# darchr/DLRM.jl

Measured on NVIDIA B200. Metric: dlrm_train_samples_per_sec, higher is better.
Workload: dtype f32 (3xTF32 interaction forward)

## Files before the change

### dlrm_jl_b200/_lib.py

```python
from __future__ import annotations

import ctypes as C
import os
from typing import Optional

HERE = os.path.dirname(os.path.abspath(__file__))
LIB_PATH = os.path.join(HERE, "lib", "libdlrm_b200.so")

OK, EINVAL, ECUDA, ENOMEM, EOOB, ESTATE, ENCCL = 0, 1, 2, 3, 4, 5, 6
_STATUS_NAMES = {EINVAL: "DLRMB_EINVAL", ECUDA: "DLRMB_ECUDA", ENOMEM: "DLRMB_ENOMEM",
                 EOOB: "DLRMB_EOOB", ESTATE: "DLRMB_ESTATE", ENCCL: "DLRMB_ENCCL"}


class DLRMB200Error(RuntimeError):
    def __init__(self, status: int, message: str):
        super().__init__(f"{_STATUS_NAMES.get(status, status)}: {message}")
        self.status = status


_i32, _i64, _f32, _vp = C.c_int32, C.c_int64, C.c_float, C.c_void_p
_idx_args = [_vp, _i32, _i32, _i32, _i32]
_idx_mp_args = [_vp, _i32, _i32, _i32, C.POINTER(_i32)]

SIGNATURES = {
    "dlrmb_abi_version": (_i32, []),
    "dlrmb_last_error": (C.c_char_p, []),
    "dlrmb_launch_count": (_i64, []),
    "dlrmb_set_option": (_i32, [C.c_char_p, _i64]),
    "dlrmb_get_option": (_i32, [C.c_char_p, C.POINTER(_i64)]),
    "dlrmb_clock_buffer_bytes": (_i64, []),
    "dlrmb_clock_kernels": (_i32, []),
    "dlrmb_clock_enable": (_i32, [_vp]),
    "dlrmb_tables_create": (_i32, [_i32, _i32, C.POINTER(_i64), _i32, _i64, C.POINTER(_vp)]),
    "dlrmb_tables_create_ex": (_i32, [_i32, _i32, C.POINTER(_i64), _i32, _i64, _i32, C.POINTER(_vp)]),
    "dlrmb_tables_elem_bytes": (_i32, [_vp]),
    "dlrmb_tables_reserve": (_i32, [_vp, _i64]),
    "dlrmb_tables_destroy": (_i32, [_vp]),
    "dlrmb_tables_info": (_i32, [_vp, C.POINTER(_i32), C.POINTER(_i32), C.POINTER(_i64), C.POINTER(_i64)]),
    "dlrmb_tables_upload": (_i32, [_vp, _i32, _vp]),
    "dlrmb_tables_download": (_i32, [_vp, _i32, _vp]),
    "dlrmb_tables_device_ptr": (_i32, [_vp, _i32, C.POINTER(_vp)]),
    "dlrmb_tables_init_uniform": (_i32, [_vp, C.c_uint64, _vp]),
    "dlrmb_tables_sync": (_i32, [_vp]),
    "dlrmb_embedding_fwd": (_i32, [_vp, *_idx_args, _vp, _i32, _i32, _vp]),
    "dlrmb_embedding_fwd_sort": (_i32, [_vp, *_idx_args, _vp, _i32, _i32, _vp]),
    "dlrmb_interaction_fwd": (_i32, [_i32, _vp, _vp, _i32, _i32, _i32, _i32, _vp, _vp]),
    "dlrmb_interaction_bwd": (_i32, [_i32, _vp, _vp, _i32, _i32, _i32, _i32, _vp, _vp, _vp]),
    "dlrmb_embedding_sort": (_i32, [_vp, *_idx_args, _vp]),
    "dlrmb_embedding_update_sorted": (_i32, [_vp, _vp, _i32, _i32, _f32, _vp]),
    "dlrmb_embedding_bwd_sgd": (_i32, [_vp, *_idx_args, _vp, _i32, _i32, _f32, _vp]),
    "dlrmb_sort_dedup_export": (_i32, [_vp, _i32, _vp, _vp, _vp, C.POINTER(_i32)]),
    "dlrmb_check_indices": (_i32, [_vp, *_idx_args, _i32]),
    "dlrmb_bce_sigmoid_fwd_bwd": (_i32, [_i32, _vp, _vp, _i32, _vp, _vp, _vp, _vp, _vp]),
    "dlrmb_xbuf_create": (_i32, [_i32, _i64, C.POINTER(_vp)]),
    "dlrmb_xbuf_destroy": (_i32, [_vp]),
    "dlrmb_xbuf_ptr": (_i32, [_vp, C.POINTER(_vp)]),
    "dlrmb_xbuf_ipc_handle": (_i32, [_vp, _vp]),
    "dlrmb_xbuf_open": (_i32, [_i32, _vp, C.POINTER(_vp)]),
    "dlrmb_xbuf_close": (_i32, [_i32, _vp]),
    "dlrmb_tables_set_slot_map": (_i32, [_vp, C.POINTER(_i32)]),
    "dlrmb_tables_set_dest_map": (_i32, [_vp, C.POINTER(_i32), C.POINTER(_i32), _i32]),
    "dlrmb_embedding_fwd_p2p": (_i32, [_vp, *_idx_args, C.POINTER(_vp), _i32, _i32, _i32, _vp]),
    "dlrmb_embedding_fwd_p2p_sort": (_i32, [_vp, *_idx_args, C.POINTER(_vp), _i32, _i32, _i32, _vp]),
    "dlrmb_embedding_fwd_p2p_mp": (_i32, [_vp, *_idx_mp_args, C.POINTER(_vp), _i32, _i32, _i32, _vp]),
    "dlrmb_embedding_fwd_p2p_sort_mp": (_i32, [_vp, *_idx_mp_args, C.POINTER(_vp), _i32, _i32, _i32, _vp]),
    "dlrmb_peer_barrier": (_i32, [_i32, C.POINTER(_vp), _i32, _i32, _i32, _vp, _vp]),
    "dlrmb_peer_barrier_flag_bytes": (_i64, []),
    "dlrmb_peer_barrier_state_bytes": (_i64, []),
    "dlrmb_peer_allreduce_f32": (_i32, [_i32, C.POINTER(_vp), C.POINTER(_vp), _i32, _i32, _i32, _vp, _vp, _i64, _vp]),
    "dlrmb_indices_scatter_p2p": (_i32, [_i32, _vp, _i32, _i32, _i32, _i32, _vp, _i32, _vp]),
    "dlrmb_indices_scatter_p2p_mp": (_i32, [_i32, _vp, _i32, _i32, _i32, C.POINTER(_i32), _vp, _i32, _vp]),
    "dlrmb_indices_scatter_p2p_mp_list": (_i32, [_i32, _vp, _i32, _i32, _i32, C.POINTER(_i32), _i32, C.POINTER(_i32),
                                                 _vp, _i32, _vp]),
    "dlrmb_interaction_has_warp_path": (_i32, [_i32, _i32]),
    "dlrmb_dense_fwd_bias_act": (_i32, [_i32, _vp, _vp, _i32, _i32, _i32, _vp]),
    "dlrmb_dense_bwd_scratch_floats": (_i64, [_i32]),
    "dlrmb_dense_bwd_act_bias": (_i32, [_i32, _vp, _vp, _i32, _i32, _vp, _vp, _vp, _vp]),
    "dlrmb_interaction_bwd_scatter": (_i32, [_i32, _vp, _vp, _i32, _i32, _i32, _i32, _vp, _i64, _vp, _vp]),
    "dlrmb_interaction_bwd_scatter_cols": (_i32, [_i32, _vp, _vp, _i32, _i32, _i32, _i32, _vp, _i32, _i64, _vp, _vp]),
    "dlrmb_interaction_bwd_dx": (_i32, [_i32, _vp, _vp, _i32, _i32, _i32, _i32, _vp, _vp]),
    "dlrmb_dac_unpack": (_i32, [_i32, _vp, _i32, _vp, _vp, _vp, _vp]),
    "dlrmb_shard_plan": (_i32, [_i32, C.POINTER(_i64), _i32, C.POINTER(_i32)]),
    "dlrmb_shard_plan_mp": (_i32, [_i32, C.POINTER(_i64), C.POINTER(_i32), _i32, C.POINTER(_i32)]),
    "dlrmb_shard_plan_cw": (_i32, [_i32, C.POINTER(_i64), C.POINTER(_i32), _i32, _i32, _i32, C.POINTER(_i32),
                                   C.POINTER(_i32)]),
    "dlrmb_comm_unique_id": (_i32, [_vp]),
    "dlrmb_comm_create": (_i32, [_i32, _vp, _i32, _i32, C.POINTER(_vp)]),
    "dlrmb_comm_destroy": (_i32, [_vp]),
    "dlrmb_comm_info": (_i32, [_vp, C.POINTER(_i32), C.POINTER(_i32)]),
    "dlrmb_comm_a2a_indices": (_i32, [_vp, C.POINTER(_i32), _i32, _vp, _i32, _i32, _i32, _vp, _vp]),
    "dlrmb_comm_a2a_indices_mp": (_i32, [_vp, C.POINTER(_i32), _i32, _vp, _i32, _i32, C.POINTER(_i32), _vp, _vp]),
    "dlrmb_comm_a2a_fwd": (_i32, [_vp, C.POINTER(_i32), _i32, _vp, _i32, _i32, _vp, _vp]),
    "dlrmb_comm_a2a_bwd": (_i32, [_vp, C.POINTER(_i32), _i32, _vp, _i32, _i32, _vp, _vp]),
    "dlrmb_comm_allreduce_f32": (_i32, [_vp, _vp, _i64, _vp]),
    "dlrmb_comm_allgather": (_i32, [_vp, _vp, _vp, _i64, _vp]),
    "dlrmb_embedding_fwd_host": (_i32, [_vp, *_idx_args, _vp, _i32, _i32]),
    "dlrmb_interaction_fwd_host": (_i32, [_vp, _vp, _vp, _i32, _i32, _i32, _i32, _vp]),
    "dlrmb_interaction_bwd_host": (_i32, [_vp, _vp, _vp, _i32, _i32, _i32, _i32, _vp, _vp]),
    "dlrmb_embedding_bwd_sgd_host": (_i32, [_vp, *_idx_args, _vp, _i32, _i32, _f32]),
    "dlrmb_mp_max_tables": (_i32, []),
    "dlrmb_embedding_fwd_mp": (_i32, [_vp, *_idx_mp_args, _vp, _i32, _i32, _vp]),
    "dlrmb_embedding_fwd_sort_mp": (_i32, [_vp, *_idx_mp_args, _vp, _i32, _i32, _vp]),
    "dlrmb_embedding_sort_mp": (_i32, [_vp, *_idx_mp_args, _vp]),
    "dlrmb_embedding_bwd_sgd_mp": (_i32, [_vp, *_idx_mp_args, _vp, _i32, _i32, _f32, _vp]),
    "dlrmb_check_indices_mp": (_i32, [_vp, *_idx_mp_args, _i32]),
    "dlrmb_embedding_fwd_mp_host": (_i32, [_vp, *_idx_mp_args, _vp, _i32, _i32]),
    "dlrmb_embedding_bwd_sgd_mp_host": (_i32, [_vp, *_idx_mp_args, _vp, _i32, _i32, _f32]),
}

_lib: Optional[C.CDLL] = None


def load() -> C.CDLL:
    global _lib
    if _lib is not None:
        return _lib
    if not os.path.exists(LIB_PATH):
        raise DLRMB200Error(
            ESTATE,
            f"{LIB_PATH} not found: build it with `python -m dlrm_jl_b200.csrc.build` "
            "(there is no CPU or PyTorch fallback for this path)")
    lib = C.CDLL(LIB_PATH)
    for name, (res, args) in SIGNATURES.items():
        fn = getattr(lib, name)
        fn.restype = res
        fn.argtypes = args
    if lib.dlrmb_abi_version() != 1:
        raise DLRMB200Error(ESTATE, f"ABI version mismatch: library has {lib.dlrmb_abi_version()}, binding expects 1")
    _lib = lib
    return lib
# ... 21 lines not shown
```

### dlrm_jl_b200/csrc/api.cu

```cuda
#include <stdarg.h>
#include <stdlib.h>
#include <string.h>

#include <mutex>

#include "common.cuh"

namespace dlrmb {

static thread_local char tl_error[512] = "";
std::atomic<long long> g_launches{0};
Options g_opt;
static std::atomic<unsigned long long*> g_clock_buf{nullptr};
unsigned long long* clock_slot(int which) {
    unsigned long long* b = g_clock_buf.load(std::memory_order_relaxed);
    return b ? b + (size_t)which * 2 * kClockCtas : nullptr;
}

void set_error(const char* fmt, ...) {
    va_list ap;
    va_start(ap, fmt);
    vsnprintf(tl_error, sizeof(tl_error), fmt, ap);
    va_end(ap);
}
// ... 339 lines not shown
    return run_uniform(t, idx, idx_bytes, B, P, slot0, true, [&](dlrmb_tables* v, const void* gidx, const MpGeom& g, int gslot0) {
        return launch_lookup_sort_mp(v, gidx, idx_bytes, idx_base, g, out, slots, gslot0, (cudaStream_t)stream);
    });
}

static int check_interaction_args(int B, int F, int d, int pad_to_mul) {
    DLRMB_REQUIRE(B > 0 && F >= 1 && d >= 1, "B, F, d must be positive (got %d, %d, %d)", B, F, d);
    DLRMB_REQUIRE(F <= 255, "F = %d exceeds 255 feature slots", F);
    DLRMB_REQUIRE(pad_to_mul >= 1, "pad_to_mul must be >= 1 (got %d)", pad_to_mul);
    return DLRMB_OK;
}

int32_t dlrmb_interaction_fwd(int32_t device, float* T, const float* x, int32_t B, int32_t F,
                              int32_t d, int32_t pad_to_mul, float* out, dlrmb_stream stream) {
    int rc = check_interaction_args(B, F, d, pad_to_mul);
    if (rc) return rc;
    DLRMB_REQUIRE(T != nullptr && out != nullptr, "T / out is null");
    DeviceGuard guard(device);
    DLRMB_REQUIRE(guard.ok, "cudaSetDevice(%d) failed", device);
    return launch_interaction_fwd(T, x, B, F, d, pad_to_mul, out, device_sm_count(device), (cudaStream_t)stream);
}

int32_t dlrmb_interaction_bwd(int32_t device, const float* dOut, const float* T, int32_t B,
                              int32_t F, int32_t d, int32_t pad_to_mul, float* dT, float* dx,
                              dlrmb_stream stream) {
    int rc = check_interaction_args(B, F, d, pad_to_mul);
    if (rc) return rc;
    DLRMB_REQUIRE(dOut && T && dT && dx, "null buffer");
    DeviceGuard guard(device);
    DLRMB_REQUIRE(guard.ok, "cudaSetDevice(%d) failed", device);
    return launch_interaction_bwd(dOut, T, B, F, d, pad_to_mul, dT, dx, device_sm_count(device), (cudaStream_t)stream);
}

int32_t dlrmb_dense_fwd_bias_act(int32_t device, float* z, const float* bias, int32_t B, int32_t N, int32_t relu,
                                 dlrmb_stream stream) {
    DLRMB_REQUIRE(B > 0 && N > 0, "B and N must be positive (got %d, %d)", B, N);
    DLRMB_REQUIRE(z && bias, "null buffer");
    DeviceGuard guard(device);
    DLRMB_REQUIRE(guard.ok, "cudaSetDevice(%d) failed", device);
    return launch_dense_fwd_bias_act(z, bias, B, N, relu, device_sm_count(device), (cudaStream_t)stream);
}

int64_t dlrmb_dense_bwd_scratch_floats(int32_t N) { return dense_bwd_scratch_floats(N); }

int32_t dlrmb_dense_bwd_act_bias(int32_t device, const float* dy, const float* y, int32_t B, int32_t N,
                                 float* dz, float* db, float* scratch, dlrmb_stream stream) {
    DLRMB_REQUIRE(B > 0 && N > 0, "B and N must be positive (got %d, %d)", B, N);
    DLRMB_REQUIRE(dy && dz && db && scratch, "null buffer");
    DeviceGuard guard(device);
    DLRMB_REQUIRE(guard.ok, "cudaSetDevice(%d) failed", device);
    return launch_dense_bwd_act_bias(dy, y, B, N, dz, db, scratch, (cudaStream_t)stream);
}

int32_t dlrmb_interaction_has_warp_path(int32_t F, int32_t d) { return interaction_has_warp_path(F, d) ? 1 : 0; }

int32_t dlrmb_interaction_bwd_scatter(int32_t device, const float* dOut, const float* T, int32_t B,
                                      int32_t F, int32_t d, int32_t pad_to_mul,
                                      const dlrmb_slot_dest* dests, int64_t sample_offset, float* dx,
                                      dlrmb_stream stream) {
    int rc = check_interaction_args(B, F, d, pad_to_mul);
    if (rc) return rc;
    DLRMB_REQUIRE(dOut && T && dests && dx, "null buffer");
    DeviceGuard guard(device);
    DLRMB_REQUIRE(guard.ok, "cudaSetDevice(%d) failed", device);
    return launch_interaction_bwd_ex(dOut, T, B, F, d, pad_to_mul, const_cast<float*>(T) , dx, dests,
                                     (long long)sample_offset, 0, device_sm_count(device), (cudaStream_t)stream);
}

int32_t dlrmb_interaction_bwd_scatter_cols(int32_t device, const float* dOut, const float* T, int32_t B,
                                           int32_t F, int32_t d, int32_t pad_to_mul, const dlrmb_slot_dest* dests,
                                           int32_t Q, int64_t sample_offset, float* dx, dlrmb_stream stream) {
    int rc = check_interaction_args(B, F, d, pad_to_mul);
    if (rc) return rc;
    DLRMB_REQUIRE(dOut && T && dests && dx, "null buffer");
    DLRMB_REQUIRE(Q >= 1 && Q <= 32 && (Q & (Q - 1)) == 0, "Q must be a power of two in 1..32 (got %d)", Q);
    DLRMB_REQUIRE(d % Q == 0 && (d / Q) % 4 == 0, "d / Q must be a multiple of 4 (d = %d, Q = %d)", d, Q);
    int qlog = 0;
    while ((1 << qlog) < Q) ++qlog;
    DeviceGuard guard(device);
    DLRMB_REQUIRE(guard.ok, "cudaSetDevice(%d) failed", device);
    return launch_interaction_bwd_ex(dOut, T, B, F, d, pad_to_mul, const_cast<float*>(T) , dx, dests,
                                     (long long)sample_offset, qlog, device_sm_count(device), (cudaStream_t)stream);
}

int32_t dlrmb_interaction_bwd_dx(int32_t device, const float* dOut, const float* T, int32_t B, int32_t F, int32_t d,
                                 int32_t pad_to_mul, float* dx, dlrmb_stream stream) {
    int rc = check_interaction_args(B, F, d, pad_to_mul);
    if (rc) return rc;
    DLRMB_REQUIRE(dOut && T && dx, "null buffer");
    DeviceGuard guard(device);
    DLRMB_REQUIRE(guard.ok, "cudaSetDevice(%d) failed", device);
    return launch_interaction_bwd_dx(dOut, T, B, F, d, pad_to_mul, dx, device_sm_count(device), (cudaStream_t)stream);
}

int32_t dlrmb_embedding_sort(dlrmb_tables* t, const void* idx, int32_t idx_bytes, int32_t idx_base,
                             int32_t B, int32_t P, dlrmb_stream stream) {
    GUARD(t);
    int rc = check_idx_args(t, idx, idx_bytes, idx_base, B, P);
    if (rc) return rc;
    t->sorted_valid = false;
    return run_uniform(t, idx, idx_bytes, B, P, 0, true, [&](dlrmb_tables* v, const void* gidx, const MpGeom& g, int) {
        return launch_sort_mp(v, gidx, idx_bytes, idx_base, g, 0, sort_mp_final_half(v, g), (cudaStream_t)stream);
    });
}

int32_t dlrmb_embedding_update_sorted(dlrmb_tables* t, const float* dT, int32_t slots,
// ... 371 lines not shown
```

### dlrm_jl_b200/csrc/build.py

```python
from __future__ import annotations

import os
import shutil
import subprocess
import sys

HERE = os.path.dirname(os.path.abspath(__file__))
ROOT = os.path.dirname(os.path.dirname(HERE))
LIB_DIR = os.path.join(os.path.dirname(HERE), "lib")
LIB_PATH = os.path.join(LIB_DIR, "libdlrm_b200.so")
SOURCES = ["api.cu", "lookup.cu", "interact.cu", "interact_warp.cu", "sort.cu", "update.cu", "loss.cu", "dense.cu", "p2p.cu", "loader.cu", "comm.cu"]
HEADERS = [os.path.join(HERE, "common.cuh"), os.path.join(HERE, "sort_small.cuh"), os.path.join(ROOT, "include", "dlrm_b200.h")]
NVCC_FLAGS = [
    "-gencode", "arch=compute_100a,code=sm_100a",
    "-O3", "-std=c++17", "-lineinfo",
    "-Xcompiler", "-fPIC,-O3,-Wall,-Wno-unused-function",
    "-I", os.path.join(ROOT, "include"), "-I", HERE,
]


def _nvcc() -> str:
    cand = shutil.which("nvcc") or "/usr/local/cuda/bin/nvcc"
    if not os.path.exists(cand):
        raise RuntimeError("nvcc not found: libdlrm_b200.so cannot be built")
    return cand


def needs_build() -> bool:
    if not os.path.exists(LIB_PATH):
        return True
    t = os.path.getmtime(LIB_PATH)
    deps = [os.path.join(HERE, s) for s in SOURCES] + HEADERS
    return any(os.path.getmtime(d) > t for d in deps)


def build(force: bool = False, verbose: bool = False) -> str:
    if not force and not needs_build():
        return LIB_PATH
    os.makedirs(LIB_DIR, exist_ok=True)
    obj_dir = os.path.join(LIB_DIR, "obj")
    os.makedirs(obj_dir, exist_ok=True)
    nvcc = _nvcc()
    procs = []
    objs = []
    for src in SOURCES:
        obj = os.path.join(obj_dir, src.replace(".cu", ".o"))
        objs.append(obj)
        cmd = [nvcc, *NVCC_FLAGS, "-c", os.path.join(HERE, src), "-o", obj]
        if verbose:
            cmd.insert(1, "-Xptxas=-v")
            print(" ".join(cmd), flush=True)
        procs.append((src, subprocess.Popen(cmd, stdout=subprocess.PIPE, stderr=subprocess.STDOUT, text=True)))
    failed = False
    for src, p in procs:
        out, _ = p.communicate()
        if p.returncode != 0:
            failed = True
            sys.stderr.write(f"--- nvcc failed on {src} ---\n{out}\n")
        elif verbose or out.strip():
            sys.stderr.write(out)
    if failed:
        raise RuntimeError("nvcc compilation failed")
    cmd = [nvcc, "-shared", "-o", LIB_PATH, *objs, "-gencode", "arch=compute_100a,code=sm_100a", "-lcudart", "-ldl"]
    subprocess.run(cmd, check=True)
# ... 6 lines not shown
```

### dlrm_jl_b200/csrc/common.cuh

```cuda
#pragma once
#include <cuda_bf16.h>
#include <cuda_runtime.h>
#include <stdint.h>
#include <stdio.h>
#include <string.h>

#include <type_traits>

#include <atomic>

#include "dlrm_b200.h"

namespace dlrmb {

void set_error(const char* fmt, ...);
extern std::atomic<long long> g_launches;

#define DLRMB_CUDA(expr)                                                                    \
    do {                                                                                    \
        cudaError_t _e = (expr);                                                            \
        if (_e != cudaSuccess) {                                                            \
            ::dlrmb::set_error("%s failed at %s:%d: %s", #expr, __FILE__, __LINE__,         \
                               cudaGetErrorString(_e));                                     \
            return (_e == cudaErrorMemoryAllocation) ? DLRMB_ENOMEM : DLRMB_ECUDA;          \
// ... 143 lines not shown
    cudaStream_t own_stream = nullptr;

    uint32_t* keys[2] = {nullptr, nullptr};
    uint32_t* pos[2] = {nullptr, nullptr};
    uint32_t* tile_hist = nullptr;
    uint32_t* digit_total = nullptr;
    int sorted_buf = 0;
    int64_t radix_tiles_cap = 0;
    float* partial = nullptr;
    uint8_t* tile_flags = nullptr;
    int64_t partial_tiles_cap = 0;
    uint32_t* head_list = nullptr;
    uint32_t* head_count = nullptr;
    int32_t* d_seg = nullptr;
    int64_t* d_uniq = nullptr;
    int32_t* d_nuniq = nullptr;

    bool sorted_valid = false;
    int sorted_B = 0;
    int32_t* h_sorted_P = nullptr;

    void* stage_idx = nullptr;  size_t stage_idx_bytes = 0;
    float* stage_a = nullptr;   size_t stage_a_bytes = 0;
    float* stage_b = nullptr;   size_t stage_b_bytes = 0;
    float* stage_c = nullptr;   size_t stage_c_bytes = 0;
    float* stage_d = nullptr;   size_t stage_d_bytes = 0;
};

namespace dlrmb {

int launch_interaction_fwd(float* T, const float* x, int B, int F, int d, int pad_to_mul,
                           float* out, int sm_count, cudaStream_t s);
int launch_interaction_bwd(const float* dOut, const float* T, int B, int F, int d, int pad_to_mul,
                           float* dT, float* dx, int sm_count, cudaStream_t s);
int launch_interaction_bwd_ex(const float* dOut, const float* T, int B, int F, int d, int pad_to_mul,
                              float* dT, float* dx, const void* dests, long long sample_offset, int qlog,
                              int sm_count, cudaStream_t s);
int launch_interaction_bwd_dx(const float* dOut, const float* T, int B, int F, int d, int pad_to_mul, float* dx,
                              int sm_count, cudaStream_t s);
bool interaction_has_warp_path(int F, int d);
int launch_update(dlrmb_tables* t, const float* dT, int slots, int slot0, float lr, cudaStream_t s);
int launch_dedup_export(dlrmb_tables* t, int k, cudaStream_t s);
int launch_init_uniform(dlrmb_tables* t, uint64_t seed, cudaStream_t s);
int launch_convert_rows(dlrmb_tables* t, int k, float* f32_buf, bool to_table, cudaStream_t s);
int launch_check_indices(dlrmb_tables* t, const void* d_idx, int idx_bytes, int idx_base, int B,
                         int P, cudaStream_t s, long long* bad_table, long long* bad_pos,
                         long long* bad_val);
int launch_bce_sigmoid(const float* z, const float* y, int B, float* prob, float* dz, float* loss,
                       float* scratch, cudaStream_t s);
int launch_dense_fwd_bias_act(float* z, const float* bias, int B, int N, int relu, int sm_count, cudaStream_t s);
int64_t dense_bwd_scratch_floats(int N);
int launch_dense_bwd_act_bias(const float* dy, const float* y, int B, int N, float* dz, float* db,
                              float* scratch, cudaStream_t s);
int launch_lookup_mp(dlrmb_tables* t, const void* idx, int idx_bytes, int idx_base, const MpGeom& g,
                     float* out, int slots, int slot0, cudaStream_t s);
int launch_lookup_sort_mp(dlrmb_tables* t, const void* idx, int idx_bytes, int idx_base, const MpGeom& g,
                          float* out, int slots, int slot0, cudaStream_t s);
int launch_sort_mp(dlrmb_tables* t, const void* idx, int idx_bytes, int idx_base, const MpGeom& g, int64_t skip_max,
                   int half, cudaStream_t s);
int sort_mp_final_half(const dlrmb_tables* t, const MpGeom& g);
int launch_update_mp(dlrmb_tables* t, const float* dT, int slots, int slot0, float lr, cudaStream_t s);
int launch_check_indices_mp(dlrmb_tables* t, const void* d_idx, int idx_bytes, int idx_base, const MpGeom& g,
                            cudaStream_t s, long long* bad_table, long long* bad_pos, long long* bad_val);
int check_mp_args(const dlrmb_tables* t, const void* idx, int idx_bytes, int idx_base, int B, const int32_t* P,
                  MpGeom* g);
void mark_sorted(dlrmb_tables* t, const MpGeom& g, int k0);
dlrmb_tables table_group(const dlrmb_tables& t, int k0, int n);
int64_t lookup_grid_mp(const dlrmb_tables* t, MpGeom& g, uint32_t C, int* cshift);
static inline int64_t sorted_lookups(const dlrmb_tables* t, int k) { return (int64_t)t->sorted_B * t->h_sorted_P[k]; }

template <typename Launch>
int run_uniform(dlrmb_tables* t, const void* idx, int idx_bytes, int B, int P, int slot0, bool sorts, Launch&& launch) {
    MpGeom g;
    g.B = (uint32_t)B;
    g.nlist = 0;
    for (int k = 0; k < kMpMaxTables; ++k) {
        g.P[k] = (uint32_t)P;
        g.off[k] = (int64_t)k * B * P;
    }
    for (int k0 = 0; k0 < t->ntab; k0 += kMpMaxTables) {
        g.ntab = t->ntab - k0 < kMpMaxTables ? t->ntab - k0 : kMpMaxTables;
        dlrmb_tables v = table_group(*t, k0, g.ntab);
        int rc = launch(&v, static_cast<const char*>(idx) + (size_t)k0 * B * P * idx_bytes, g, slot0 + k0);
        if (rc) return rc;
        if (sorts) {
            t->sorted_buf = v.sorted_buf;
            mark_sorted(t, g, k0);
        }
    }
    return DLRMB_OK;
}
int device_sm_count(int device);
int64_t update_tiles_cap(int ntab, int D, int64_t max_lookups, int sm_count);
int ensure_smem_attr(const void* func, int bytes, unsigned long long* done_mask);

static inline int64_t ceil_div64(int64_t a, int64_t b) { return (a + b - 1) / b; }

}
```

### dlrm_jl_b200/dense.py

```python
from __future__ import annotations

from typing import List, Optional, Sequence

import torch
from torch import nn

from . import _lib


def _stream(t: torch.Tensor) -> int:
    return int(torch.cuda.current_stream(t.device).cuda_stream)


class _DenseFn(torch.autograd.Function):

    @staticmethod
    def forward(ctx, x: torch.Tensor, weight: torch.Tensor, bias: torch.Tensor, relu: bool,
                gw: torch.Tensor, gb: torch.Tensor, scratch: torch.Tensor):
        if not x.is_cuda:
            raise _lib.DLRMB200Error(_lib.EINVAL, "fused dense layers run on the GPU only (no CPU fallback)")
        x = x.contiguous()
        y = torch.mm(x, weight.t())
        _lib.check(_lib.load().dlrmb_dense_fwd_bias_act(
            y.device.index or 0, y.data_ptr(), bias.data_ptr(), y.shape[0], y.shape[1], 1 if relu else 0, _stream(y)))
        ctx.relu = relu
        ctx.gw, ctx.gb, ctx.scratch = gw, gb, scratch
        ctx.save_for_backward(x, weight, y if relu else None)
        return y

    @staticmethod
    def backward(ctx, dy: torch.Tensor):
        x, weight, y = ctx.saved_tensors
        dy = dy.contiguous()
        B, N = dy.shape
        dz = torch.empty_like(dy) if ctx.relu else dy
        _lib.check(_lib.load().dlrmb_dense_bwd_act_bias(
            dy.device.index or 0, dy.data_ptr(), y.data_ptr() if ctx.relu else None, B, N, dz.data_ptr(),
            ctx.gb.data_ptr(), ctx.scratch.data_ptr(), _stream(dy)))
        torch.mm(dz.t(), x, out=ctx.gw)
        dx = dz @ weight if ctx.needs_input_grad[0] else None
        return dx, None, None, None, None, None, None


class FusedDense(nn.Module):

    def __init__(self, linear: nn.Linear, relu: bool, grad_weight: Optional[torch.Tensor] = None,
                 grad_bias: Optional[torch.Tensor] = None):
        super().__init__()
        self.linear = linear
        self.relu = relu
        dev = linear.weight.device
        self.grad_weight = grad_weight if grad_weight is not None else torch.zeros_like(linear.weight)
        self.grad_bias = grad_bias if grad_bias is not None else torch.zeros_like(linear.bias)
        assert self.grad_weight.is_contiguous() and self.grad_weight.shape == linear.weight.shape
        assert self.grad_bias.is_contiguous() and self.grad_bias.shape == linear.bias.shape
        n = int(_lib.load().dlrmb_dense_bwd_scratch_floats(linear.out_features))
        self.scratch = torch.zeros(n, dtype=torch.float32, device=dev)

    def forward(self, x: torch.Tensor) -> torch.Tensor:
        return _DenseFn.apply(x, self.linear.weight, self.linear.bias, self.relu, self.grad_weight,
                              self.grad_bias, self.scratch)


class FusedMLP(nn.Module):

    def __init__(self, seq: Sequence[nn.Module], grads: Optional[Sequence[torch.Tensor]] = None):
        super().__init__()
        mods = list(seq)
        layers: List[nn.Module] = []
        gi = 0
        i = 0
        while i < len(mods):
            lin = mods[i]
            assert isinstance(lin, nn.Linear), "expected Linear (+ activation) pairs"
            act = mods[i + 1] if i + 1 < len(mods) and not isinstance(mods[i + 1], nn.Linear) else None
            gw = grads[gi] if grads is not None else None
            gb = grads[gi + 1] if grads is not None else None
            gi += 2
            layers.append(FusedDense(lin, isinstance(act, nn.ReLU), gw, gb))
            if act is not None and not isinstance(act, nn.ReLU):
                layers.append(act)
            i += 1 if act is None else 2
        self.layers = nn.Sequential(*layers)

    def forward(self, x: torch.Tensor) -> torch.Tensor:
        return self.layers(x)

    def bind_param_grads(self) -> None:
        for m in self.layers:
            if isinstance(m, FusedDense):
                m.linear.weight.grad = m.grad_weight
                m.linear.bias.grad = m.grad_bias

    def grad_buffers(self) -> List[torch.Tensor]:
        out = []
        for m in self.layers:
            if isinstance(m, FusedDense):
                out += [m.grad_weight, m.grad_bias]
        return out


__all__ = ["FusedDense", "FusedMLP"]
```

### include/dlrm_b200.h

```cpp
#ifndef DLRM_B200_H
#define DLRM_B200_H

#include <stdint.h>

#ifdef __cplusplus
extern "C" {
#endif

typedef struct dlrmb_tables dlrmb_tables;
typedef void* dlrmb_stream;

typedef enum dlrmb_status {
    DLRMB_OK = 0,
    DLRMB_EINVAL = 1,
    DLRMB_ECUDA = 2,
    DLRMB_ENOMEM = 3,
    DLRMB_EOOB = 4,
    DLRMB_ESTATE = 5,
    DLRMB_ENCCL = 6
} dlrmb_status;

#define DLRMB_ABI_VERSION 1

int32_t dlrmb_abi_version(void);
// ... 25 lines not shown
                            dlrmb_stream stream);

int32_t dlrmb_embedding_fwd_sort(dlrmb_tables* t, const void* idx, int32_t idx_bytes, int32_t idx_base,
                                 int32_t B, int32_t P, float* out, int32_t slots, int32_t slot0,
                                 dlrmb_stream stream);

int32_t dlrmb_interaction_fwd(int32_t device, float* T, const float* x, int32_t B, int32_t F,
                              int32_t d, int32_t pad_to_mul, float* out, dlrmb_stream stream);
int32_t dlrmb_interaction_bwd(int32_t device, const float* dOut, const float* T, int32_t B,
                              int32_t F, int32_t d, int32_t pad_to_mul, float* dT, float* dx,
                              dlrmb_stream stream);
int32_t dlrmb_interaction_has_warp_path(int32_t F, int32_t d);

int32_t dlrmb_embedding_sort(dlrmb_tables* t, const void* idx, int32_t idx_bytes, int32_t idx_base,
                             int32_t B, int32_t P, dlrmb_stream stream);
int32_t dlrmb_embedding_update_sorted(dlrmb_tables* t, const float* dT, int32_t slots,
                                      int32_t slot0, float lr, dlrmb_stream stream);
int32_t dlrmb_embedding_bwd_sgd(dlrmb_tables* t, const void* idx, int32_t idx_bytes,
                                int32_t idx_base, int32_t B, int32_t P, const float* dT,
                                int32_t slots, int32_t slot0, float lr, dlrmb_stream stream);

int32_t dlrmb_sort_dedup_export(dlrmb_tables* t, int32_t k, int64_t* uniq, int32_t* seg_offsets,
                                int32_t* perm, int32_t* n_uniq);
int32_t dlrmb_check_indices(dlrmb_tables* t, const void* idx, int32_t idx_bytes, int32_t idx_base,
                            int32_t B, int32_t P, int32_t idx_on_host);

int32_t dlrmb_mp_max_tables(void);
int32_t dlrmb_embedding_fwd_mp(dlrmb_tables* t, const void* idx, int32_t idx_bytes, int32_t idx_base, int32_t B,
                               const int32_t* P, float* out, int32_t slots, int32_t slot0, dlrmb_stream stream);
int32_t dlrmb_embedding_fwd_sort_mp(dlrmb_tables* t, const void* idx, int32_t idx_bytes, int32_t idx_base, int32_t B,
                                    const int32_t* P, float* out, int32_t slots, int32_t slot0, dlrmb_stream stream);
int32_t dlrmb_embedding_sort_mp(dlrmb_tables* t, const void* idx, int32_t idx_bytes, int32_t idx_base, int32_t B,
                                const int32_t* P, dlrmb_stream stream);
int32_t dlrmb_embedding_bwd_sgd_mp(dlrmb_tables* t, const void* idx, int32_t idx_bytes, int32_t idx_base, int32_t B,
                                   const int32_t* P, const float* dT, int32_t slots, int32_t slot0, float lr,
                                   dlrmb_stream stream);
int32_t dlrmb_check_indices_mp(dlrmb_tables* t, const void* idx, int32_t idx_bytes, int32_t idx_base, int32_t B,
                               const int32_t* P, int32_t idx_on_host);
int32_t dlrmb_embedding_fwd_mp_host(dlrmb_tables* t, const void* idx, int32_t idx_bytes, int32_t idx_base, int32_t B,
                                    const int32_t* P, float* out, int32_t slots, int32_t slot0);
int32_t dlrmb_embedding_bwd_sgd_mp_host(dlrmb_tables* t, const void* idx, int32_t idx_bytes, int32_t idx_base,
                                        int32_t B, const int32_t* P, const float* dT, int32_t slots, int32_t slot0,
                                        float lr);

int32_t dlrmb_bce_sigmoid_fwd_bwd(int32_t device, const float* logits, const float* labels, int32_t B,
                                  float* prob, float* dlogits, float* loss, float* scratch,
                                  dlrmb_stream stream);

int32_t dlrmb_dense_fwd_bias_act(int32_t device, float* z, const float* bias, int32_t B, int32_t N, int32_t relu,
                                 dlrmb_stream stream);
int64_t dlrmb_dense_bwd_scratch_floats(int32_t N);
int32_t dlrmb_dense_bwd_act_bias(int32_t device, const float* dy, const float* y, int32_t B, int32_t N,
                                 float* dz, float* db, float* scratch, dlrmb_stream stream);

int32_t dlrmb_dac_unpack(int32_t device, const void* records, int32_t B, float* labels, float* dense,
                         uint32_t* sparse, dlrmb_stream stream);

typedef struct dlrmb_xbuf dlrmb_xbuf;
int32_t dlrmb_xbuf_create(int32_t device, int64_t bytes, dlrmb_xbuf** out);
int32_t dlrmb_xbuf_destroy(dlrmb_xbuf* x);
int32_t dlrmb_xbuf_ptr(dlrmb_xbuf* x, void** dev);
int32_t dlrmb_xbuf_ipc_handle(dlrmb_xbuf* x, uint8_t* handle64);
int32_t dlrmb_xbuf_open(int32_t device, const uint8_t* handle64, void** peer_ptr);
int32_t dlrmb_xbuf_close(int32_t device, void* peer_ptr);
int32_t dlrmb_tables_set_slot_map(dlrmb_tables* t, const int32_t* slots);
int32_t dlrmb_tables_set_dest_map(dlrmb_tables* t, const int32_t* slots, const int32_t* col0, int32_t D_dest);
int32_t dlrmb_embedding_fwd_p2p(dlrmb_tables* t, const void* idx, int32_t idx_bytes, int32_t idx_base,
                                int32_t B_global, int32_t P, float* const* peer_T, int32_t world,
                                int32_t B_local, int32_t slots, dlrmb_stream stream);

int32_t dlrmb_embedding_fwd_p2p_sort(dlrmb_tables* t, const void* idx, int32_t idx_bytes, int32_t idx_base,
                                     int32_t B_global, int32_t P, float* const* peer_T, int32_t world,
                                     int32_t B_local, int32_t slots, dlrmb_stream stream);
int32_t dlrmb_embedding_fwd_p2p_mp(dlrmb_tables* t, const void* idx, int32_t idx_bytes, int32_t idx_base,
                                   int32_t B_global, const int32_t* P, float* const* peer_T, int32_t world,
                                   int32_t B_local, int32_t slots, dlrmb_stream stream);
int32_t dlrmb_embedding_fwd_p2p_sort_mp(dlrmb_tables* t, const void* idx, int32_t idx_bytes, int32_t idx_base,
                                        int32_t B_global, const int32_t* P, float* const* peer_T, int32_t world,
                                        int32_t B_local, int32_t slots, dlrmb_stream stream);

int32_t dlrmb_peer_barrier(int32_t device, uint32_t* const* peer_flags, int32_t world, int32_t rank, int32_t channel,
                           uint32_t* state, dlrmb_stream stream);
int64_t dlrmb_peer_barrier_flag_bytes(void);
int64_t dlrmb_peer_barrier_state_bytes(void);
int32_t dlrmb_peer_allreduce_f32(int32_t device, float* const* peer_bufs, uint32_t* const* peer_flags, int32_t world,
                                 int32_t rank, int32_t channel, uint32_t* state, float* data, int64_t n,
                                 dlrmb_stream stream);
int32_t dlrmb_indices_scatter_p2p(int32_t device, const void* idx_local, int32_t idx_bytes, int32_t ntab,
                                  int32_t B_local, int32_t P, const void* const* dests_dev, int32_t rank,
                                  dlrmb_stream stream);
int32_t dlrmb_indices_scatter_p2p_mp(int32_t device, const void* idx_local, int32_t idx_bytes, int32_t ntab,
                                     int32_t B_local, const int32_t* P, const void* const* dests_dev, int32_t rank,
                                     dlrmb_stream stream);
int32_t dlrmb_indices_scatter_p2p_mp_list(int32_t device, const void* idx_local, int32_t idx_bytes, int32_t ntab,
                                          int32_t B_local, const int32_t* P, int32_t ndest, const int32_t* dest_table,
                                          const void* const* dests_dev, int32_t rank, dlrmb_stream stream);

typedef struct dlrmb_slot_dest {
    float* base;
    int64_t sample_stride;
    int64_t offset;
} dlrmb_slot_dest;
int32_t dlrmb_interaction_bwd_scatter(int32_t device, const float* dOut, const float* T, int32_t B,
                                      int32_t F, int32_t d, int32_t pad_to_mul,
                                      const dlrmb_slot_dest* dests, int64_t sample_offset, float* dx,
                                      dlrmb_stream stream);
// ... 44 lines not shown
```

Baseline: 2.324 million.

## Add 3xTF32 tcgen05 GEMM kernel for dense MLP forward, dgrad and wgrad

Adds a custom Blackwell GEMM that splits fp32 operands into TF32 hi/lo parts and runs three tcgen05 MMAs per k-slice. Warps are specialized into loaders, an MMA issuer and TMEM accumulator readers, and bias and ReLU are fused into the epilogue. The Python dense layer sends large enough shapes to this kernel instead of torch.mm and the separate bias/act kernel. The aim is to replace FP32 cuBLAS GEMMs with tensor-core work while keeping near-fp32 accuracy. The risks are slower non-TMA, register-based loads and per-k-tile accumulation round-trips through TMEM.

```diff
diff --git a/dlrm_jl_b200/_lib.py b/dlrm_jl_b200/_lib.py
--- a/dlrm_jl_b200/_lib.py
+++ b/dlrm_jl_b200/_lib.py
@@ -76,6 +76,9 @@
     "dlrmb_dense_fwd_bias_act": (_i32, [_i32, _vp, _vp, _i32, _i32, _i32, _vp]),
     "dlrmb_dense_bwd_scratch_floats": (_i64, [_i32]),
     "dlrmb_dense_bwd_act_bias": (_i32, [_i32, _vp, _vp, _i32, _i32, _vp, _vp, _vp, _vp]),
+    "dlrmb_dense_fwd": (_i32, [_i32, _vp, _vp, _vp, _i32, _i32, _i32, _i32, _vp, _vp]),
+    "dlrmb_dense_dgrad": (_i32, [_i32, _vp, _vp, _i32, _i32, _i32, _vp, _vp]),
+    "dlrmb_dense_wgrad": (_i32, [_i32, _vp, _vp, _i32, _i32, _i32, _vp, _vp]),
     "dlrmb_interaction_bwd_scatter": (_i32, [_i32, _vp, _vp, _i32, _i32, _i32, _i32, _vp, _i64, _vp, _vp]),
     "dlrmb_interaction_bwd_scatter_cols": (_i32, [_i32, _vp, _vp, _i32, _i32, _i32, _i32, _vp, _i32, _i64, _vp, _vp]),
     "dlrmb_interaction_bwd_dx": (_i32, [_i32, _vp, _vp, _i32, _i32, _i32, _i32, _vp, _vp]),
diff --git a/dlrm_jl_b200/csrc/api.cu b/dlrm_jl_b200/csrc/api.cu
--- a/dlrm_jl_b200/csrc/api.cu
+++ b/dlrm_jl_b200/csrc/api.cu
@@ -415,6 +415,33 @@
     return launch_dense_bwd_act_bias(dy, y, B, N, dz, db, scratch, (cudaStream_t)stream);
 }
 
+int32_t dlrmb_dense_fwd(int32_t device, const float* x, const float* w, const float* bias, int32_t B, int32_t in,
+                        int32_t out, int32_t relu, float* y, dlrmb_stream stream) {
+    DLRMB_REQUIRE(B > 0 && in > 0 && out > 0, "B, in and out must be positive (got %d, %d, %d)", B, in, out);
+    DLRMB_REQUIRE(x && w && y, "null buffer");
+    DeviceGuard guard(device);
+    DLRMB_REQUIRE(guard.ok, "cudaSetDevice(%d) failed", device);
+    return launch_dense_fwd(x, w, bias, B, in, out, relu, y, (cudaStream_t)stream);
+}
+
+int32_t dlrmb_dense_dgrad(int32_t device, const float* dz, const float* w, int32_t B, int32_t in, int32_t out,
+                          float* dx, dlrmb_stream stream) {
+    DLRMB_REQUIRE(B > 0 && in > 0 && out > 0, "B, in and out must be positive (got %d, %d, %d)", B, in, out);
+    DLRMB_REQUIRE(dz && w && dx, "null buffer");
+    DeviceGuard guard(device);
+    DLRMB_REQUIRE(guard.ok, "cudaSetDevice(%d) failed", device);
+    return launch_dense_dgrad(dz, w, B, in, out, dx, (cudaStream_t)stream);
+}
+
+int32_t dlrmb_dense_wgrad(int32_t device, const float* dz, const float* x, int32_t B, int32_t in, int32_t out,
+                          float* dw, dlrmb_stream stream) {
+    DLRMB_REQUIRE(B > 0 && in > 0 && out > 0, "B, in and out must be positive (got %d, %d, %d)", B, in, out);
+    DLRMB_REQUIRE(dz && x && dw, "null buffer");
+    DeviceGuard guard(device);
+    DLRMB_REQUIRE(guard.ok, "cudaSetDevice(%d) failed", device);
+    return launch_dense_wgrad(dz, x, B, in, out, dw, (cudaStream_t)stream);
+}
+
 int32_t dlrmb_interaction_has_warp_path(int32_t F, int32_t d) { return interaction_has_warp_path(F, d) ? 1 : 0; }
 
 int32_t dlrmb_interaction_bwd_scatter(int32_t device, const float* dOut, const float* T, int32_t B,
diff --git a/dlrm_jl_b200/csrc/build.py b/dlrm_jl_b200/csrc/build.py
--- a/dlrm_jl_b200/csrc/build.py
+++ b/dlrm_jl_b200/csrc/build.py
@@ -9,7 +9,7 @@
 ROOT = os.path.dirname(os.path.dirname(HERE))
 LIB_DIR = os.path.join(os.path.dirname(HERE), "lib")
 LIB_PATH = os.path.join(LIB_DIR, "libdlrm_b200.so")
-SOURCES = ["api.cu", "lookup.cu", "interact.cu", "interact_warp.cu", "sort.cu", "update.cu", "loss.cu", "dense.cu", "p2p.cu", "loader.cu", "comm.cu"]
+SOURCES = ["api.cu", "lookup.cu", "interact.cu", "interact_warp.cu", "sort.cu", "update.cu", "loss.cu", "dense.cu", "dense_gemm.cu", "p2p.cu", "loader.cu", "comm.cu"]
 HEADERS = [os.path.join(HERE, "common.cuh"), os.path.join(HERE, "sort_small.cuh"), os.path.join(ROOT, "include", "dlrm_b200.h")]
 NVCC_FLAGS = [
     "-gencode", "arch=compute_100a,code=sm_100a",
diff --git a/dlrm_jl_b200/csrc/common.cuh b/dlrm_jl_b200/csrc/common.cuh
--- a/dlrm_jl_b200/csrc/common.cuh
+++ b/dlrm_jl_b200/csrc/common.cuh
@@ -219,6 +219,10 @@
 int64_t dense_bwd_scratch_floats(int N);
 int launch_dense_bwd_act_bias(const float* dy, const float* y, int B, int N, float* dz, float* db,
                               float* scratch, cudaStream_t s);
+int launch_dense_fwd(const float* x, const float* w, const float* bias, int B, int in, int out, int relu, float* y,
+                     cudaStream_t s);
+int launch_dense_dgrad(const float* dz, const float* w, int B, int in, int out, float* dx, cudaStream_t s);
+int launch_dense_wgrad(const float* dz, const float* x, int B, int in, int out, float* dw, cudaStream_t s);
 int launch_lookup_mp(dlrmb_tables* t, const void* idx, int idx_bytes, int idx_base, const MpGeom& g,
                      float* out, int slots, int slot0, cudaStream_t s);
 int launch_lookup_sort_mp(dlrmb_tables* t, const void* idx, int idx_bytes, int idx_base, const MpGeom& g,
diff --git a/dlrm_jl_b200/csrc/dense_gemm.cu b/dlrm_jl_b200/csrc/dense_gemm.cu
--- /dev/null
+++ b/dlrm_jl_b200/csrc/dense_gemm.cu
@@ -0,0 +1,344 @@
+#include "common.cuh"
+
+namespace dlrmb {
+
+namespace {
+
+constexpr int kBM = 128, kBN = 128, kBK = 32, kStages = 3;
+constexpr int kLoadWarps = 8, kLoadThreads = kLoadWarps * 32;
+constexpr int kAccWarps = 4;
+constexpr int kThreads = kLoadThreads + kAccWarps * 32 + 32;
+constexpr int kTasks = (kBM / 8) * 2 / kLoadWarps;
+constexpr int kOpBytes = kBM * kBK * 4;
+constexpr int kStageBytes = 4 * kOpBytes;
+constexpr int kSmemBytes = kStages * kStageBytes + 128;
+constexpr uint32_t kLBO = (kBM / 8) * 128;
+constexpr uint32_t kSBO = 128;
+constexpr int kTmemCols = 4 * kBN;
+constexpr uint32_t kIdesc = (1u << 4) | (2u << 7) | (2u << 10) | ((uint32_t)(kBN >> 3) << 17) |
+                            ((uint32_t)(kBM >> 4) << 24);
+static_assert(kTasks * kLoadWarps * 32 == kBM * kBK / 4, "loader tasks must cover the tile");
+static_assert(kLoadWarps % 4 == 0, "accumulator warp w must sit on TMEM lane quarter w % 4");
+
+struct Operand {
+    const float* p;
+    long long ld;
+    int vec;
+};
+
+struct GemmArgs {
+    Operand a, b;
+    int M, N, K;
+    float* c;
+    long long ldc;
+    const float* bias;
+    int relu;
+};
+
+__device__ __forceinline__ uint32_t smem_u32(const void* p) { return (uint32_t)__cvta_generic_to_shared(p); }
+
+__device__ __forceinline__ uint64_t make_desc(uint32_t saddr) {
+    uint64_t d = 0;
+    d |= (uint64_t)((saddr & 0x3FFFFu) >> 4);
+    d |= (uint64_t)((kLBO >> 4) & 0x3FFFu) << 16;
+    d |= (uint64_t)((kSBO >> 4) & 0x3FFFu) << 32;
+    d |= (uint64_t)1 << 46;
+    return d;
+}
+
+__device__ __forceinline__ void mbar_init(uint64_t* b, int count) {
+    asm volatile("mbarrier.init.shared::cta.b64 [%0], %1;\n" ::"r"(smem_u32(b)), "r"(count));
+}
+__device__ __forceinline__ void mbar_arrive(uint64_t* b) {
+    asm volatile("mbarrier.arrive.shared::cta.b64 _, [%0];\n" ::"r"(smem_u32(b)) : "memory");
+}
+__device__ __forceinline__ void mbar_wait(uint64_t* b, uint32_t parity) {
+    uint32_t done = 0;
+    while (!done) {
+        asm volatile("{\n .reg .pred p;\n mbarrier.try_wait.parity.shared::cta.b64 p, [%1], %2;\n selp.u32 %0, 1, 0, p;\n}\n"
+                     : "=r"(done) : "r"(smem_u32(b)), "r"(parity) : "memory");
+    }
+}
+
+__device__ __forceinline__ uint32_t rna_tf32(float x) {
+    uint32_t r;
+    asm("cvt.rna.tf32.f32 %0, %1;" : "=r"(r) : "f"(x));
+    return r;
+}
+
+__device__ __forceinline__ void split_store(uint32_t hi_addr, uint32_t lo_addr, float4 v) {
+    const uint32_t h0 = rna_tf32(v.x), h1 = rna_tf32(v.y), h2 = rna_tf32(v.z), h3 = rna_tf32(v.w);
+    const uint32_t l0 = rna_tf32(v.x - __uint_as_float(h0)), l1 = rna_tf32(v.y - __uint_as_float(h1));
+    const uint32_t l2 = rna_tf32(v.z - __uint_as_float(h2)), l3 = rna_tf32(v.w - __uint_as_float(h3));
+    asm volatile("st.shared.v4.b32 [%0], {%1, %2, %3, %4};\n" ::"r"(hi_addr), "r"(h0), "r"(h1), "r"(h2), "r"(h3) : "memory");
+    asm volatile("st.shared.v4.b32 [%0], {%1, %2, %3, %4};\n" ::"r"(lo_addr), "r"(l0), "r"(l1), "r"(l2), "r"(l3) : "memory");
+}
+
+template <bool KMAJOR>
+__device__ __forceinline__ void task_rc(int warp, int lane, int i, int& r, int& c) {
+    const int t = warp + kLoadWarps * i;
+    if (KMAJOR) {
+        r = 8 * (t & 15) + (lane & 7);
+        c = 4 * (t >> 4) + (lane >> 3);
+    } else {
+        r = 32 * (t & 3) + lane;
+        c = t >> 2;
+    }
+}
+
+template <bool KMAJOR>
+__device__ __forceinline__ float4 load_chunk(const Operand& op, int gr, int rows, int k, int K) {
+    float4 v = make_float4(0.f, 0.f, 0.f, 0.f);
+    if (gr >= rows || k >= K) return v;
+    if (KMAJOR) {
+        const float* q = op.p + (size_t)gr * op.ld + k;
+        if (op.vec) return __ldg(reinterpret_cast<const float4*>(q));
+        v.x = __ldg(q);
+        if (k + 1 < K) v.y = __ldg(q + 1);
+        if (k + 2 < K) v.z = __ldg(q + 2);
+        if (k + 3 < K) v.w = __ldg(q + 3);
+    } else {
+        const float* q = op.p + (size_t)k * op.ld + gr;
+        v.x = __ldg(q);
+        if (k + 1 < K) v.y = __ldg(q + op.ld);
+        if (k + 2 < K) v.z = __ldg(q + 2 * op.ld);
+        if (k + 3 < K) v.w = __ldg(q + 3 * op.ld);
+    }
+    return v;
+}
+
+__device__ __forceinline__ void mma_tf32(uint32_t d_tmem, uint64_t a_desc, uint64_t b_desc, uint32_t acc) {
+    asm volatile("{\n .reg .pred p;\n setp.ne.b32 p, %4, 0;\n"
+                 " tcgen05.mma.cta_group::1.kind::tf32 [%0], %1, %2, %3, p;\n}\n"
+                 ::"r"(d_tmem), "l"(a_desc), "l"(b_desc), "r"(kIdesc), "r"(acc) : "memory");
+}
+
+__device__ __forceinline__ void mma_commit(uint64_t* bar) {
+    asm volatile("tcgen05.commit.cta_group::1.mbarrier::arrive::one.shared::cluster.b64 [%0];\n" ::"r"(smem_u32(bar)) : "memory");
+}
+
+__device__ __forceinline__ void tmem_ld32(uint32_t taddr, uint32_t (&v)[32]) {
+    asm volatile(
+        "tcgen05.ld.sync.aligned.32x32b.x32.b32 {%0, %1, %2, %3, %4, %5, %6, %7, %8, %9, %10, %11, %12, %13, %14, %15, "
+        "%16, %17, %18, %19, %20, %21, %22, %23, %24, %25, %26, %27, %28, %29, %30, %31}, [%32];\n"
+        : "=r"(v[0]), "=r"(v[1]), "=r"(v[2]), "=r"(v[3]), "=r"(v[4]), "=r"(v[5]), "=r"(v[6]), "=r"(v[7]),
+          "=r"(v[8]), "=r"(v[9]), "=r"(v[10]), "=r"(v[11]), "=r"(v[12]), "=r"(v[13]), "=r"(v[14]), "=r"(v[15]),
+          "=r"(v[16]), "=r"(v[17]), "=r"(v[18]), "=r"(v[19]), "=r"(v[20]), "=r"(v[21]), "=r"(v[22]), "=r"(v[23]),
+          "=r"(v[24]), "=r"(v[25]), "=r"(v[26]), "=r"(v[27]), "=r"(v[28]), "=r"(v[29]), "=r"(v[30]), "=r"(v[31])
+        : "r"(taddr));
+}
+
+__device__ __forceinline__ void tmem_st32(uint32_t taddr, const uint32_t (&v)[32]) {
+    asm volatile(
+        "tcgen05.st.sync.aligned.32x32b.x32.b32 [%0], {%1, %2, %3, %4, %5, %6, %7, %8, %9, %10, %11, %12, %13, %14, %15, "
+        "%16, %17, %18, %19, %20, %21, %22, %23, %24, %25, %26, %27, %28, %29, %30, %31, %32};\n"
+        ::"r"(taddr), "r"(v[0]), "r"(v[1]), "r"(v[2]), "r"(v[3]), "r"(v[4]), "r"(v[5]), "r"(v[6]), "r"(v[7]),
+          "r"(v[8]), "r"(v[9]), "r"(v[10]), "r"(v[11]), "r"(v[12]), "r"(v[13]), "r"(v[14]), "r"(v[15]),
+          "r"(v[16]), "r"(v[17]), "r"(v[18]), "r"(v[19]), "r"(v[20]), "r"(v[21]), "r"(v[22]), "r"(v[23]),
+          "r"(v[24]), "r"(v[25]), "r"(v[26]), "r"(v[27]), "r"(v[28]), "r"(v[29]), "r"(v[30]), "r"(v[31])
+        : "memory");
+}
+
+__device__ __forceinline__ void store_slice(const GemmArgs& g, float* stg, const uint32_t (&x)[32], int q, int c,
+                                            int lane, int m0, int n0) {
+#pragma unroll
+    for (int i = 0; i < 32; ++i) stg[lane * 33 + i] = __uint_as_float(x[i]);
+    __syncwarp();
+    const int col = n0 + 32 * c + lane;
+    if (col < g.N) {
+        const float bias_v = g.bias != nullptr ? __ldg(g.bias + col) : 0.f;
+        for (int i = 0; i < 32; ++i) {
+            const int row = m0 + 32 * q + i;
+            if (row >= g.M) break;
+            float v = stg[i * 33 + lane];
+            if (g.bias != nullptr) v += bias_v;
+            if (g.relu) v = fmaxf(v, 0.f);
+            g.c[(size_t)row * g.ldc + col] = v;
+        }
+    }
+    __syncwarp();
+}
+
+template <bool A_KMAJOR, bool B_KMAJOR>
+__global__ void __launch_bounds__(kThreads, 1)
+dense_gemm_kernel(const GemmArgs g) {
+    extern __shared__ uint8_t smem_raw[];
+    __shared__ __align__(8) uint64_t full_bar[kStages], empty_bar[kStages], acc_full[2], acc_empty[2];
+    __shared__ uint32_t tmem_base_s;
+    uint8_t* smem = reinterpret_cast<uint8_t*>((reinterpret_cast<uintptr_t>(smem_raw) + 127) & ~uintptr_t(127));
+    const uint32_t smem0 = smem_u32(smem);
+
+    const int tid = threadIdx.x, warp = tid >> 5, lane = tid & 31;
+    const int m0 = blockIdx.y * kBM, n0 = blockIdx.x * kBN;
+    const int nloc = (g.K + kBK - 1) / kBK, kt0 = 0;
+    const bool acc_warp = warp >= kLoadWarps && warp < kLoadWarps + kAccWarps;
+    const int q = warp & 3;
+    float* stg = reinterpret_cast<float*>(smem) + (warp - kLoadWarps) * 32 * 33;
+
+    if (warp == 0) {
+        asm volatile("tcgen05.alloc.cta_group::1.sync.aligned.shared::cta.b32 [%0], %1;\n" ::"r"(smem_u32(&tmem_base_s)), "r"(kTmemCols));
+        asm volatile("tcgen05.relinquish_alloc_permit.cta_group::1.sync.aligned;\n");
+    }
+    if (tid == 0) {
+        for (int s = 0; s < kStages; ++s) {
+            mbar_init(&full_bar[s], kLoadThreads);
+            mbar_init(&empty_bar[s], 1);
+        }
+        for (int b = 0; b < 2; ++b) {
+            mbar_init(&acc_full[b], 1);
+            mbar_init(&acc_empty[b], kAccWarps * 32);
+        }
+        asm volatile("fence.mbarrier_init.release.cluster;\n" ::: "memory");
+    }
+    asm volatile("tcgen05.fence::before_thread_sync;\n" ::: "memory");
+    __syncthreads();
+    asm volatile("tcgen05.fence::after_thread_sync;\n" ::: "memory");
+    const uint32_t tmem = tmem_base_s;
+
+    if (warp < kLoadWarps) {
+        int ar[kTasks], ac[kTasks], br[kTasks], bc[kTasks];
+#pragma unroll
+        for (int i = 0; i < kTasks; ++i) {
+            task_rc<A_KMAJOR>(warp, lane, i, ar[i], ac[i]);
+            task_rc<B_KMAJOR>(warp, lane, i, br[i], bc[i]);
+        }
+        float4 ra[kTasks], rb[kTasks];
+#pragma unroll
+        for (int i = 0; i < kTasks; ++i) {
+            ra[i] = load_chunk<A_KMAJOR>(g.a, m0 + ar[i], g.M, kt0 * kBK + 4 * ac[i], g.K);
+            rb[i] = load_chunk<B_KMAJOR>(g.b, n0 + br[i], g.N, kt0 * kBK + 4 * bc[i], g.K);
+        }
+        for (int j = 0; j < nloc; ++j) {
+            float4 na[kTasks], nb[kTasks];
+            const bool more = j + 1 < nloc;
+            const int kn = (kt0 + j + 1) * kBK;
+#pragma unroll
+            for (int i = 0; i < kTasks; ++i) {
+                na[i] = more ? load_chunk<A_KMAJOR>(g.a, m0 + ar[i], g.M, kn + 4 * ac[i], g.K) : make_float4(0.f, 0.f, 0.f, 0.f);
+                nb[i] = more ? load_chunk<B_KMAJOR>(g.b, n0 + br[i], g.N, kn + 4 * bc[i], g.K) : make_float4(0.f, 0.f, 0.f, 0.f);
+            }
+            const int s = j % kStages;
+            if (j >= kStages) mbar_wait(&empty_bar[s], ((j / kStages) + 1) & 1);
+            const uint32_t st = smem0 + s * kStageBytes;
+#pragma unroll
+            for (int i = 0; i < kTasks; ++i) {
+                const uint32_t oa = ac[i] * kLBO + ar[i] * 16, ob = bc[i] * kLBO + br[i] * 16;
+                split_store(st + oa, st + kOpBytes + oa, ra[i]);
+                split_store(st + 2 * kOpBytes + ob, st + 3 * kOpBytes + ob, rb[i]);
+            }
+            asm volatile("fence.proxy.async.shared::cta;\n" ::: "memory");
+            mbar_arrive(&full_bar[s]);
+#pragma unroll
+            for (int i = 0; i < kTasks; ++i) { ra[i] = na[i]; rb[i] = nb[i]; }
+        }
+    } else if (acc_warp) {
+        const uint32_t lanes = (uint32_t)(32 * q) << 16;
+        for (int j = 0; j < nloc; ++j) {
+            const int b = j & 1;
+            const bool last = j == nloc - 1;
+            mbar_wait(&acc_full[b], (j >> 1) & 1);
+            asm volatile("tcgen05.fence::after_thread_sync;\n" ::: "memory");
+#pragma unroll 1
+            for (int c = 0; c < kBN / 32; ++c) {
+                uint32_t v[32], sum[32];
+                tmem_ld32(tmem + lanes + b * kBN + 32 * c, v);
+                if (j > 0) tmem_ld32(tmem + lanes + 2 * kBN + 32 * c, sum);
+                asm volatile("tcgen05.wait::ld.sync.aligned;\n" ::: "memory");
+#pragma unroll
+                for (int i = 0; i < 32; ++i)
+                    sum[i] = j > 0 ? __float_as_uint(__uint_as_float(sum[i]) + __uint_as_float(v[i])) : v[i];
+                if (last) store_slice(g, stg, sum, q, c, lane, m0, n0);
+                else tmem_st32(tmem + lanes + 2 * kBN + 32 * c, sum);
+            }
+            if (!last) asm volatile("tcgen05.wait::st.sync.aligned;\n" ::: "memory");
+            asm volatile("tcgen05.fence::before_thread_sync;\n" ::: "memory");
+            mbar_arrive(&acc_empty[b]);
+        }
+    } else if (warp == kLoadWarps + kAccWarps) {
+        for (int j = 0; j < nloc; ++j) {
+            const int s = j % kStages, b = j & 1;
+            mbar_wait(&full_bar[s], (j / kStages) & 1);
+            if (j >= 2) mbar_wait(&acc_empty[b], ((j >> 1) + 1) & 1);
+            asm volatile("tcgen05.fence::after_thread_sync;\n" ::: "memory");
+            if (lane == 0) {
+                const uint32_t st = smem0 + s * kStageBytes;
+                const uint32_t d = tmem + b * kBN;
+#pragma unroll
+                for (int kk = 0; kk < kBK / 8; ++kk) {
+                    const uint32_t off = kk * 2 * kLBO;
+                    const uint64_t a_hi = make_desc(st + off), a_lo = make_desc(st + kOpBytes + off);
+                    const uint64_t b_hi = make_desc(st + 2 * kOpBytes + off), b_lo = make_desc(st + 3 * kOpBytes + off);
+                    mma_tf32(d, a_lo, b_hi, kk > 0 ? 1u : 0u);
+                    mma_tf32(d, a_hi, b_lo, 1u);
+                    mma_tf32(d, a_hi, b_hi, 1u);
+                }
+                mma_commit(&empty_bar[s]);
+                mma_commit(&acc_full[b]);
+            }
+            __syncwarp();
+        }
+    }
+
+    asm volatile("tcgen05.fence::before_thread_sync;\n" ::: "memory");
+    __syncthreads();
+    if (warp == 0) {
+        asm volatile("tcgen05.fence::after_thread_sync;\n" ::: "memory");
+        asm volatile("tcgen05.dealloc.cta_group::1.sync.aligned.b32 %0, %1;\n" ::"r"(tmem), "r"(kTmemCols));
+    }
+}
+
+template <bool AK, bool BK>
+int launch(const GemmArgs& g, cudaStream_t s) {
+    auto kern = dense_gemm_kernel<AK, BK>;
+    static std::atomic<uint64_t> opted_in{0};
+    int dev = 0;
+    DLRMB_CUDA(cudaGetDevice(&dev));
+    const uint64_t bit = uint64_t(1) << (dev & 63);
+    if (!(opted_in.load() & bit)) {
+        DLRMB_CUDA(cudaFuncSetAttribute(kern, cudaFuncAttributeMaxDynamicSharedMemorySize, kSmemBytes));
+        opted_in.fetch_or(bit);
+    }
+    dim3 grid((unsigned)((g.N + kBN - 1) / kBN), (unsigned)((g.M + kBM - 1) / kBM));
+    kern<<<grid, kThreads, kSmemBytes, s>>>(g);
+    DLRMB_LAUNCH_CHECK();
+    return DLRMB_OK;
+}
+
+Operand operand(const float* p, long long ld, bool kmajor, int K) {
+    const bool vec = kmajor && ld % 4 == 0 && K % 4 == 0 && (reinterpret_cast<uintptr_t>(p) & 15) == 0;
+    return Operand{p, ld, vec ? 1 : 0};
+}
+
+GemmArgs args(int M, int N, int K, float* c, const float* bias, int relu) {
+    GemmArgs g{};
+    g.M = M; g.N = N; g.K = K;
+    g.c = c; g.ldc = N;
+    g.bias = bias; g.relu = relu;
+    return g;
+}
+
+}
+
+int launch_dense_fwd(const float* x, const float* w, const float* bias, int B, int in, int out, int relu, float* y,
+                     cudaStream_t s) {
+    GemmArgs g = args(B, out, in, y, bias, relu);
+    g.a = operand(x, in, true, in);
+    g.b = operand(w, in, true, in);
+    return launch<true, true>(g, s);
+}
+
+int launch_dense_dgrad(const float* dz, const float* w, int B, int in, int out, float* dx, cudaStream_t s) {
+    GemmArgs g = args(B, in, out, dx, nullptr, 0);
+    g.a = operand(dz, out, true, out);
+    g.b = operand(w, in, false, out);
+    return launch<true, false>(g, s);
+}
+
+int launch_dense_wgrad(const float* dz, const float* x, int B, int in, int out, float* dw, cudaStream_t s) {
+    GemmArgs g = args(out, in, B, dw, nullptr, 0);
+    g.a = operand(dz, out, false, B);
+    g.b = operand(x, in, false, B);
+    return launch<false, false>(g, s);
+}
+
+}
diff --git a/dlrm_jl_b200/dense.py b/dlrm_jl_b200/dense.py
--- a/dlrm_jl_b200/dense.py
+++ b/dlrm_jl_b200/dense.py
@@ -12,6 +12,10 @@
     return int(torch.cuda.current_stream(t.device).cuda_stream)
 
 
+def on_tensor_cores(M: int, N: int, K: int) -> bool:
+    return -(-M // 128) * -(-N // 128) >= 128 and K >= 64
+
+
 class _DenseFn(torch.autograd.Function):
 
     @staticmethod
@@ -20,9 +24,18 @@
         if not x.is_cuda:
             raise _lib.DLRMB200Error(_lib.EINVAL, "fused dense layers run on the GPU only (no CPU fallback)")
         x = x.contiguous()
-        y = torch.mm(x, weight.t())
-        _lib.check(_lib.load().dlrmb_dense_fwd_bias_act(
-            y.device.index or 0, y.data_ptr(), bias.data_ptr(), y.shape[0], y.shape[1], 1 if relu else 0, _stream(y)))
+        B, n_in = x.shape
+        n_out = weight.shape[0]
+        dev = x.device.index or 0
+        lib = _lib.load()
+        if on_tensor_cores(B, n_out, n_in):
+            y = torch.empty((B, n_out), dtype=torch.float32, device=x.device)
+            _lib.check(lib.dlrmb_dense_fwd(dev, x.data_ptr(), weight.data_ptr(), bias.data_ptr(), B, n_in, n_out,
+                                           1 if relu else 0, y.data_ptr(), _stream(y)))
+        else:
+            y = torch.mm(x, weight.t())
+            _lib.check(lib.dlrmb_dense_fwd_bias_act(
+                dev, y.data_ptr(), bias.data_ptr(), B, n_out, 1 if relu else 0, _stream(y)))
         ctx.relu = relu
         ctx.gw, ctx.gb, ctx.scratch = gw, gb, scratch
         ctx.save_for_backward(x, weight, y if relu else None)
@@ -37,8 +50,21 @@
         _lib.check(_lib.load().dlrmb_dense_bwd_act_bias(
             dy.device.index or 0, dy.data_ptr(), y.data_ptr() if ctx.relu else None, B, N, dz.data_ptr(),
             ctx.gb.data_ptr(), ctx.scratch.data_ptr(), _stream(dy)))
-        torch.mm(dz.t(), x, out=ctx.gw)
-        dx = dz @ weight if ctx.needs_input_grad[0] else None
+        n_in = x.shape[1]
+        dev = dy.device.index or 0
+        lib = _lib.load()
+        if on_tensor_cores(N, n_in, B):
+            _lib.check(lib.dlrmb_dense_wgrad(dev, dz.data_ptr(), x.data_ptr(), B, n_in, N, ctx.gw.data_ptr(), _stream(dy)))
+        else:
+            torch.mm(dz.t(), x, out=ctx.gw)
+        dx = None
+        if ctx.needs_input_grad[0]:
+            if on_tensor_cores(B, n_in, N):
+                dx = torch.empty_like(x)
+                _lib.check(lib.dlrmb_dense_dgrad(dev, dz.data_ptr(), weight.data_ptr(), B, n_in, N, dx.data_ptr(),
+                                                 _stream(dy)))
+            else:
+                dx = dz @ weight
         return dx, None, None, None, None, None, None
 
 
@@ -56,6 +82,7 @@
         assert self.grad_bias.is_contiguous() and self.grad_bias.shape == linear.bias.shape
         n = int(_lib.load().dlrmb_dense_bwd_scratch_floats(linear.out_features))
         self.scratch = torch.zeros(n, dtype=torch.float32, device=dev)
+        assert linear.weight.is_contiguous()
 
     def forward(self, x: torch.Tensor) -> torch.Tensor:
         return _DenseFn.apply(x, self.linear.weight, self.linear.bias, self.relu, self.grad_weight,
diff --git a/include/dlrm_b200.h b/include/dlrm_b200.h
--- a/include/dlrm_b200.h
+++ b/include/dlrm_b200.h
@@ -101,6 +101,13 @@
 int64_t dlrmb_dense_bwd_scratch_floats(int32_t N);
 int32_t dlrmb_dense_bwd_act_bias(int32_t device, const float* dy, const float* y, int32_t B, int32_t N,
                                  float* dz, float* db, float* scratch, dlrmb_stream stream);
+
+int32_t dlrmb_dense_fwd(int32_t device, const float* x, const float* w, const float* bias, int32_t B, int32_t in,
+                        int32_t out, int32_t relu, float* y, dlrmb_stream stream);
+int32_t dlrmb_dense_dgrad(int32_t device, const float* dz, const float* w, int32_t B, int32_t in, int32_t out,
+                          float* dx, dlrmb_stream stream);
+int32_t dlrmb_dense_wgrad(int32_t device, const float* dz, const float* x, int32_t B, int32_t in, int32_t out,
+                          float* dw, dlrmb_stream stream);
 
 int32_t dlrmb_dac_unpack(int32_t device, const void* records, int32_t B, float* labels, float* dense,
                          uint32_t* sparse, dlrmb_stream stream);
```

New measurement: 2.500 million (median of 6 runs). 1.08x the previous value.
